# cerbos/cerbos

Measured on NVIDIA H100. Metric: checkresources_decisions_per_sec, higher is better.
Workload: dtype u64

## Files before the change

### cerbos_b200/csrc/cb_core.h

```cpp
#pragma once
#include <stdint.h>
#if !defined(__CUDACC_RTC__)
#include <math.h>
#endif

#include "cerbos_b200_format.h"

#if defined(__CUDACC__)
#define CB_HD __host__ __device__ __forceinline__
#define CB_HD_NOINLINE __host__ __device__ __noinline__
#else
#define CB_HD inline
#define CB_HD_NOINLINE
#endif

namespace cb {

struct alignas(16) U4 { uint32_t x, y, z, w; };

struct TableLayout {
    uint32_t off[32];
    uint32_t nV, nRP, nS, nP, nR, nAP, nT, n_slots, n_rows;
    uint32_t has_role_policies, has_parent_roles, has_principal_policies;
    uint32_t image_bytes;
// ... 39 lines not shown
    CB_HD const U4 *urows() const { return reinterpret_cast<const U4 *>(base + L->uc_rows_off); }
    CB_HD const U4 *uc_chain() const { return reinterpret_cast<const U4 *>(base + L->uc_chain_off); }
};

enum { CB_MAX_GATHER = 8 };
struct BatchView {
    const cb_hdr0 *hdr0;
    const cb_hdr1 *hdr1;
    const uint32_t *roles;
    const uint64_t *slots;
    const uint64_t *heap;
    const uint32_t *bstr_off;
    const uint8_t *bstr_bytes;
    const uint32_t *class_off, *class_pats, *aset_k;
    const uint64_t *aset_spread;
    const uint64_t *row_am;
    uint32_t n_rows;
    uint64_t stride;
    uint64_t first, count;
    uint32_t role_cols, n_asets, kc, n_pass, max_actions, kbytes, flags;
    uint32_t rcp, stride_pattern;
    int64_t now;
    const uint32_t *perm;
    uint32_t prefetch_slots;
    uint32_t *defer_list, *defer_count;
    uint32_t *count_dev;
    uint32_t *tile_counter;
    uint8_t *outs[CB_MAX_GATHER];
    uint32_t n_out;
    uint32_t *sig_flags[CB_MAX_GATHER];
    const uint32_t *wait_flags;
    uint32_t sig_rank, sig_step, wait_step;
    const uint32_t *strpred;
    const U4 *uc_rows_pk;
    uint32_t n_bstr;
    uint64_t heap_words;
};

#ifndef __CUDACC_RTC__
inline void finish_batch_view(BatchView &b) {
    b.perm = nullptr;
    b.prefetch_slots = 0;
    b.defer_list = nullptr; b.defer_count = nullptr; b.count_dev = nullptr; b.tile_counter = nullptr;
    b.n_out = 0;
    for (int i = 0; i < CB_MAX_GATHER; i++) { b.outs[i] = nullptr; b.sig_flags[i] = nullptr; }
    b.wait_flags = nullptr; b.sig_rank = 0; b.sig_step = 0; b.wait_step = 0;
    b.strpred = nullptr;
    b.uc_rows_pk = nullptr;
    b.rcp = 1;
    while (b.rcp < b.role_cols) b.rcp <<= 1;
    b.stride_pattern = 0;
    for (uint32_t j = 0; j * b.role_cols < 32; j++) b.stride_pattern |= 1u << (j * b.role_cols);
}
#endif

template <typename T>
CB_HD T ldg(const T *p) { return *p; }

CB_HD uint64_t ldcol64(const uint64_t *p) {
#if defined(__CUDA_ARCH__)
    uint64_t v;
    asm("ld.global.nc.L1::no_allocate.u64 %0, [%1];" : "=l"(v) : "l"(p));
    return v;
#else
    return *p;
#endif
}
CB_HD uint32_t ldcol32(const uint32_t *p) {
#if defined(__CUDA_ARCH__)
    uint32_t v;
    asm("ld.global.nc.L1::no_allocate.u32 %0, [%1];" : "=r"(v) : "l"(p));
    return v;
#else
    return *p;
#endif
}

CB_HD U4 ld16(const void *p) { return *reinterpret_cast<const U4 *>(p); }
CB_HD U4 ldcol128(const void *p) {
#if defined(__CUDA_ARCH__)
// ... 3478 lines not shown
CB_HD int strpred_tri(const BatchView &b, uint64_t x, uint32_t p) {
#ifdef CB_UC_STUB_STRPRED
    return (int)((x >> p) & 1u);
#endif
    if (v64_bad(x)) return TRI_E;
    if (v64_tag(x) != CB_V64_STRING) return TRI_E;
    return (int)((ldg(b.strpred + (uint32_t)(x & 0xFFFFFFFFu)) >> p) & 1u);
}
CB_HD bool typed_str(uint64_t x) { return (uint32_t)(x >> 32) == (uint32_t)(CB_V64_BOX_BASE | CB_V64_STRING) << 16; }
CB_HD bool typed_num(uint64_t x) { const double d = u2d(x); return v64_tag(x) == 0 && d == d; }
CB_HD bool typed_bool(uint64_t x) { return (x >> 1) == (uint64_t)(CB_V64_BOX_BASE | CB_V64_BOOL) << 47; }
CB_HD bool typed_list(const ListRegs &L, uint32_t need) {
    bool ok = L.st == 0 && L.len >= need;
#ifdef CB_LIST_KEYS64
    for (int j = 0; j < CB_LC; j++) ok &= (uint32_t)j >= L.len || (uint32_t)(L.e[j] >> 48) == (CB_V64_BOX_BASE | CB_V64_STRING);
#endif
    return ok;
}
CB_HD bool uc_typed(bool guard) {
#ifdef CB_UC_STUB_FALLBACK
    return guard || true;
#endif
    return guard;
}
CB_HD uint32_t typed_id(uint64_t key) { return (uint32_t)key; }
CB_HD uint64_t typed_box(uint32_t id) { return ((uint64_t)(CB_V64_BOX_BASE | CB_V64_STRING) << 48) | id; }
CB_HD bool typed_ord(uint32_t ci, double dx, double dy) { return ci == 2 ? dx < dy : ci == 3 ? dx <= dy : ci == 4 ? dx > dy : dx >= dy; }
CB_HD bool typed_strpred(const BatchView &b, uint32_t id, uint32_t p) {
#ifdef CB_UC_STUB_STRPRED
    return ((id >> p) & 1u) != 0;
#endif
    return ((ldg(b.strpred + id) >> p) & 1u) != 0;
}
template <typename Cols>
CB_HD ListKey list_elem_key(const TableView t, const BatchView &b, const Cols &cols, uint32_t v, const ListRegs &L, uint32_t i) {
    if (L.st == 2) return list_probe_key(elem_operand(t, b, cols.slot(v), i));
    return list_probe_key(list_elem(t, b, 0ull, L, i));
}

struct OneCols {
    uint64_t x;
    CB_HD uint64_t slot(uint32_t) const { return x; }
};
CB_HD bool term_lit(int tri, uint32_t flags) { return (flags & CB_TERM_LIT_F) ? tri == TRI_F : tri == TRI_T; }
template <typename Cols>
CB_HD uint32_t flat_dnf_inline(const TableView t, const BatchView &b, const Cols &cols, uint32_t pid, uint32_t flat_off, uint32_t info) {
    const uint32_t nt = info & 0xFFFF;
    const cb_instr *terms = t.code() + flat_off;
    bool any = false, group = true, slow = false;
    for (uint32_t i = 0; i < nt; i++) {
        const U4 w = ld16(terms + 2 * i);
        const uint32_t flags = (w.x >> 8) & 0xFF;
        group &= term_lit(term_tri(t, b, cols, pid, w, slow), flags);
        if (flags & CB_TERM_GROUP_END) { any |= group; group = true; }
    }
    if (slow) return 4u;
    return (uint32_t)(any != (bool)((info >> 24) & 1));
}
template <typename Cols>
CB_HD uint32_t cond_eval(const TableView t, const BatchView &b, const Cols &cols, uint32_t pid, uint32_t gid) {
    U4 cd = ld16(t.conds() + gid);
    if (cd.w) return flat_dnf_inline(t, b, cols, pid, cd.z, cd.w);
    return 4u;
}

CB_HD uint32_t chain_start(const TableView t, uint32_t scope, uint32_t kind_flag, bool lenient) {
// ... 804 lines not shown
```

### cerbos_b200/csrc/cb_specialize.h

```cpp
#pragma once
#include <stdint.h>

#include <cstdio>
#include <cstring>
#include <map>
#include <string>
#include <vector>

#include "cerbos_b200_format.h"

namespace cbspec {

struct Limits {
    uint32_t max_shapes = 8;
    uint32_t max_items = 96;
};

inline std::string hex(uint32_t v) {
    char buf[16];
    snprintf(buf, sizeof buf, "0x%xu", v);
    return buf;
}
inline std::string hex64(uint64_t v) {
    char buf[32];
// ... 582 lines not shown
                break;
            }
            if (op == CB_TERM_STARTS || op == CB_TERM_ENDS || op == CB_TERM_CONTAINS) {
                if (xk == CB_OPK_SLOT) want(w[1], 'S');
                if (yk == CB_OPK_SLOT) want(w[2], 'S');
                break;
            }
            if (xk == CB_OPK_SLOT && yk != CB_OPK_SLOT) want(w[1], tyy);
            if (yk == CB_OPK_SLOT && xk != CB_OPK_SLOT) want(w[2], tx);
            break;
        }
        }
    }
    for (uint32_t v = 0; v < ns && typed; v++) {
        if (slot_list[v]) want(v, 'L');
        if ((slot_used[v] || slot_list[v]) && (!ty[v] || atoms.slot_used[v])) typed = false;
    }
    auto typed_operand = [&](uint32_t kind, uint32_t v, uint32_t aux, char &k) -> std::string {
        const std::string V = std::to_string(v);
        if (kind == CB_OPK_CONST) {
            const uint64_t c = consts[v];
            k = const_type(c);
            if (k == 'S') return hex((uint32_t)c);
            if (k == 'N') return "u2d(" + hex64(c) + ")";
            if (k == 'B') return c & 1u ? "true" : "false";
            return "";
        }
        if (kind == CB_OPK_PID) { k = 'S'; return "pid"; }
        if (kind == CB_OPK_SLOT_SIZE) { k = 'N'; return "(double)cols.l" + V + ".len"; }
        if (kind == CB_OPK_SLOT_ELEM) { k = 'S'; return "typed_id(cols.l" + V + ".e[" + std::to_string(aux) + "])"; }
        k = v < ns && (ty[v] == 'S' || ty[v] == 'N' || ty[v] == 'B') ? ty[v] : 0;
        return k == 'S' ? "typed_id(cols.k" + V + ")" : k == 'N' ? "cols.d" + V : k == 'B' ? "cols.b" + V : "";
    };
    auto typed_term = [&](uint32_t q) -> std::string {
        const uint32_t *w = terms[q].data();
        const uint32_t op = w[0] & 0xFF, flags = (w[0] >> 8) & 0xFF, xk = (w[0] >> 16) & 0xFF, yk = w[0] >> 24, ci = flags & CB_TERM_CI_MASK;
        if (form[q] == 'P') return "typed_strpred(b, typed_id(cols.k" + std::to_string(w[1]) + "), " + std::to_string(pred_of[q]) + "u)";
        if (form[q] == 'L') {
            if (op == CB_TERM_IN_CS || op == CB_TERM_IN_SS || op == CB_TERM_IN) {
                if (probe_of[q] == CB_NONE32) return "";
                if (op == CB_TERM_IN_CS && const_type(consts[w[1]]) == 0) return "";
                if (op == CB_TERM_IN && xk == CB_OPK_CONST && const_type(consts[w[1]]) == 0) return "";
                return "(h" + std::to_string(w[2]) + " & " + hex(1u << probe_of[q]) + ") != 0u";
            }
            const std::string a = std::to_string(mask_of[q].first), bb = std::to_string(mask_of[q].second);
            return op == CB_TERM_SUBSET ? "m" + a + "_" + bb + " == (1u << cols.l" + a + ".len) - 1u" : "m" + a + "_" + bb + " != 0u";
        }
        char kx = 0, ky = 0;
        std::string x, y;
        switch (op) {
        case CB_TERM_EQ_SS: case CB_TERM_ORD_SS:
            x = typed_operand(CB_OPK_SLOT, w[1], 0, kx); y = typed_operand(CB_OPK_SLOT, w[2], 0, ky);
            if (!kx || kx != ky) return "";
            if (op == CB_TERM_EQ_SS) return x + " == " + y;
            return kx == 'N' ? "typed_ord(" + hex(ci) + ", " + x + ", " + y + ")" : "";
        case CB_TERM_EQ_SC: case CB_TERM_ORD_SC:
            x = typed_operand(CB_OPK_SLOT, w[1], 0, kx); y = typed_operand(CB_OPK_CONST, w[2], 0, ky);
            if (!kx || kx != ky) return "";
            if (op == CB_TERM_EQ_SC) return x + " == " + y;
            return kx == 'N' ? "typed_ord(" + hex(ci) + ", " + x + ", " + y + ")" : "";
        case CB_TERM_EQ_SP: return "typed_id(cols.k" + std::to_string(w[1]) + ") == pid";
        case CB_TERM_IN_SC: {
            const uint64_t *p = theap + (consts[w[2]] & 0xFFFFFFFFFFFFull);
            x = typed_operand(CB_OPK_SLOT, w[1], 0, kx);
            if (!kx || kx != in_const_type(q)) return "";
            std::string e;
            for (uint32_t j = 0; j < (uint32_t)p[0]; j++)
                e += std::string(j ? " | " : "") + "(" + x + " == " + (kx == 'S' ? hex((uint32_t)p[1 + j]) : "u2d(" + hex64(p[1 + j]) + ")") + ")";
            return e;
        }
        case CB_TERM_HAS: return "true";
        case CB_TERM_CMP:
            x = typed_operand(xk, w[1], w[3] & 0xFFFFu, kx); y = typed_operand(yk, w[2], w[3] >> 16, ky);
            if (!kx || !ky) return "";
            if (ci == 0) return kx == ky ? x + " == " + y : "false";
            return kx == 'N' && ky == 'N' ? "typed_ord(" + hex(ci) + ", " + x + ", " + y + ")" : "";
        case CB_TERM_STARTS: case CB_TERM_ENDS: case CB_TERM_CONTAINS:
            x = typed_operand(xk, w[1], w[3] & 0xFFFFu, kx); y = typed_operand(yk, w[2], w[3] >> 16, ky);
            if (kx != 'S' || ky != 'S') return "";
            return "str_tri(t, b, " + std::to_string(op) + "u, typed_box(" + x + "), typed_box(" + y + ")) == TRI_T";
        default: return "";
        }
    };
    std::vector<std::string> tterm(terms.size());
    for (uint32_t q = 0; q < terms.size() && typed; q++) {
        tterm[q] = typed_term(q);
        typed = !tterm[q].empty();
    }
    auto probe_key = [&](const Probe &x) -> std::string {
        const std::string V = std::to_string(x.v);
        if (x.kind == CB_OPK_CONST || x.kind == CB_OPK_PID) return "list_probe_key(" + x.value + ")";
        if (x.kind == CB_OPK_SLOT) return x.v < ns && ty[x.v] == 'S' ? "cols.k" + V : "";
        if (x.kind == CB_OPK_SLOT_ELEM) return "list_elem_key(t, b, cols, " + V + "u, cols.l" + V + ", " + std::to_string(x.aux) + "u)";
        return "";
    };
    for (const auto &pl : probes)
        for (const Probe &x : pl.second) typed &= !probe_key(x).empty();
    std::string s;
    s += "// generated by cb_specialize.h (generate_uc) from the loaded table: every distinct condition, straight-line\n";
    s += "namespace cb {\n";
    for (const std::string &a : atoms.src) s += a;
    auto reg = [&](uint32_t v) { return slot_used[v] || slot_list[v]; };
    s += "struct SpecRegs {\n    CachedCols g;\n";
    for (uint32_t v = 0; v < ns; v++)
        if (reg(v)) s += "    uint64_t s" + std::to_string(v) + ";\n";
    if (typed) {
        s += "    bool typed;   // every slot below holds the type its terms compare it as (SpecConds::load)\n";
        for (uint32_t v = 0; v < ns; v++) {
            const std::string V = std::to_string(v);
            if (ty[v] == 'S') s += "    ListKey k" + V + ";   // string: its probe key (the id when typed)\n";
            if (ty[v] == 'N') s += "    double d" + V + ";\n";
            if (ty[v] == 'B') s += "    bool b" + V + ";\n";
        }
    }
    for (uint32_t v = 0; v < ns; v++)
        if (slot_list[v]) s += "    ListRegs l" + std::to_string(v) + ";\n";
    s += "    CB_HD uint64_t slot(uint32_t v) const {\n        switch (v) {\n";
    for (uint32_t v = 0; v < ns && !typed; v++)
        if (reg(v)) s += "        case " + std::to_string(v) + "u: return s" + std::to_string(v) + ";\n";
    s += "        default: return v < " + std::to_string(ns) + "u ? g.slot(v) : (uint64_t)(CB_V64_BOX_BASE | CB_V64_ERROR) << 48;\n        }\n    }\n};\n";
    s += "struct SpecConds {\n    static constexpr uint32_t n_strpred = " + std::to_string(n_pred_bits) + "u;\n";
    s += std::string("    static constexpr int kForm = ") + (n_uconds <= 31 ? "CB_UC_FORM_MASK32" : n_uconds <= 63 ? "CB_UC_FORM_MASK64" : "CB_UC_FORM_INDEX") + ";   // how the rows name their conditions\n";
    s += "    static constexpr uint32_t kScopeRows = " + std::to_string(scope_rows) + "u;   // rows of the longest scope (cb::uc_walk)\n";
    s += std::string("    static constexpr bool kPrograms = ") + (have_atoms ? "true" : "false") + ";   // leaf programs: needs the value helpers of cb_core.h\n";
    s += "    template <typename Cols>\n    CB_HD SpecRegs load(const TableView t, const BatchView &b, const Cols &c) const {\n        SpecRegs r;\n        r.g.b = c.b; r.g.n = c.n;\n";
    for (uint32_t v = 0; v < ns; v++)
        if (reg(v)) s += "        r.s" + std::to_string(v) + " = c.slot(" + std::to_string(v) + "u);\n";
    if (typed) {
        std::string guard;
        for (uint32_t v = 0; v < ns; v++) {
            const std::string V = std::to_string(v);
            if (!reg(v)) continue;
            if (ty[v] == 'L') s += "        r.l" + V + " = list_load(t, b, r.s" + V + ");\n";
            if (ty[v] == 'S') s += "        r.k" + V + " = list_probe_key(r.s" + V + ");\n";
            if (ty[v] == 'N') s += "        r.d" + V + " = u2d(r.s" + V + ");\n";
            if (ty[v] == 'B') s += "        r.b" + V + " = (r.s" + V + " & 1u) != 0;\n";
            guard += std::string(guard.empty() ? "" : " & ") + (ty[v] == 'L' ? "typed_list(r.l" + V + ", " + std::to_string(list_need[v]) + "u)"
                                                                 : std::string(ty[v] == 'S' ? "typed_str" : ty[v] == 'N' ? "typed_num" : "typed_bool") + "(r.s" + V + ")");
        }
        s += "        r.typed = " + guard + ";\n";
    } else {
        for (uint32_t v = 0; v < ns; v++)
            if (slot_list[v]) s += "        r.l" + std::to_string(v) + " = list_load(t, b, r.s" + std::to_string(v) + ");\n";
    }
    s += "        return r;\n    }\n";
    s += "    // the predicate word of one string (pre-pass over the string dictionary; bit p = predicate p holds)\n";
    s += "    CB_HD uint32_t strpred(const TableView t, const BatchView &b, uint32_t id) const {\n";
    s += "        OneCols cols; cols.x = ((uint64_t)(CB_V64_BOX_BASE | CB_V64_STRING) << 48) | id;\n        bool slow = false; uint32_t bits = 0u; const uint32_t pid = 0u;\n";
    for (uint32_t p = 0; p < pred_terms.size(); p++) {
        const uint32_t *w = terms[pred_terms[p]].data();
        s += "        bits |= (uint32_t)(term_tri(t, b, cols, pid, U4{" + hex(w[0]) + ", 0x0u, " + hex(w[2]) + ", " + hex(w[3]) + "}, slow) == TRI_T) << " + std::to_string(p) + ";\n";
    }
    {
        bool any = false;
// ... 61 lines not shown
            continue;
        }
        const uint32_t nt = cd[3] & 0xFFFFu, negate = (cd[3] >> 24) & 1u;
        std::string &c = cond_src[u];
        c += in + "{   // distinct condition " + std::to_string(u) + "\n" + in + "    bool any = false, group = true;\n";
        std::string any, group;
        for (uint32_t i = 0; i < nt; i++) {
            const uint32_t *w = code + 2 * (cd[2] + 2 * i);
            const uint32_t flags = (w[0] >> 8) & 0xFFu;
            const uint32_t q = term_ids[{w[0] & kUseMask, w[1], w[2], w[3]}];
            c += in + "    group &= term_lit(q" + std::to_string(q) + ", " + hex(flags) + ");\n";
            group += std::string(group.empty() ? "" : " & ") + (flags & CB_TERM_LIT_F ? "!t" : "t") + std::to_string(q);
            if (flags & CB_TERM_GROUP_END) {
                c += in + "    any |= group; group = true;\n";
                any += std::string(any.empty() ? "" : " | ") + "(" + group + ")";
                group.clear();
            }
        }
        c += in + "    " + word + std::string(" |= (uint64_t)(any != ") + (negate ? "true" : "false") + ") << " + sh + ";\n" + in + "}\n";
        if (any.empty()) any = "false";
        typed_src += "            " + word + " |= (uint64_t)(" + (negate ? "!(" + any + ")" : any) + ") << " + sh + ";   // condition " + std::to_string(u) + "\n";
    }
    if (typed) {
        s += atom_src + "        CondWord val; val.lo = 1ull; val.hi = 0ull;\n" + typed_src + "        } else {   // the tri-state terms on the slot words, reloaded (cols.slot)\n" + tri;
        for (uint32_t u = 1; u <= n_uconds; u++) if (formula[u].empty()) s += cond_src[u];
        s += "        }\n";
        for (uint32_t u = 1; u <= n_uconds; u++) if (!formula[u].empty()) s += cond_src[u];
    } else {
        s += tri + atom_src + "        CondWord val; val.lo = 1ull; val.hi = 0ull;\n";
        for (uint32_t u = 1; u <= n_uconds; u++) s += cond_src[u];
    }
    s += "        return val;\n    }\n};\n}  // namespace cb\n";
    out.src = s;
    out.n_strpred = n_pred_bits;
    out.n_atoms = (uint32_t)atoms.src.size();
    return out;
}

}
```

### cerbos_b200/csrc/cerbos_b200.cu

```cuda
#include <cuda_runtime.h>
#include <dlfcn.h>
#include <sys/stat.h>
#include <unistd.h>

#include <atomic>
#include <cstdarg>
#include <cstdio>
#include <cstdlib>
#include <cstring>
#include <map>
#include <mutex>
#include <new>
#include <string>
#include <thread>
#include <vector>

#include "cb_core.h"
#include "cb_kernels.h"
#include "cb_specialize.h"
#include "cb_uc.h"
#include "cb_encode.h"
#include "cb_narrow.h"
#include "cb_host.h"
#include "cb_embed.inc"
// ... 317 lines not shown
        while (c < n) c <<= 1;
        T *fresh = nullptr;
        const cudaError_t e = cudaMallocAsync(reinterpret_cast<void **>(&fresh), c * sizeof(T), stream);
        if (e != cudaSuccess) return e;
        T *old = ptr;
        ptr = fresh;
        cap = c;
        return old ? cudaFreeAsync(old, stream) : cudaSuccess;
    }
};

}

struct cgpu_ctx {
    int device = 0;
    int sm_count = 0;
    uint32_t *d_status = nullptr;
    std::atomic<uint64_t> launches{0};
    std::mutex mu;
    std::vector<Slot> slots;
    LaunchPlan last_plan;
    uint32_t last_grid = 0, last_window = 0, last_buckets = 0;
    int force_no_stage = 0;
    int force_general = 0;
    int cluster_mode = -1;
    int force_no_tiles = 0;
    int force_no_jit = 0;
    struct DeferLane {
        uint32_t seq = 0;
        uint32_t *cells = nullptr;
        struct Bufs {
            LaneBuf<uint32_t> list;
            LaneBuf<uint32_t> strpred;
            LaneBuf<cb::U4> pk;
        } q[4];
    };
    std::map<cudaStream_t, DeferLane> defer_lanes;
    std::mutex defer_mu;
    cudaStream_t copy_stream = nullptr;
    cudaEvent_t copy_ev[16] = {};
    uint32_t copy_seq = 0;
    struct SliceUse { const void *ptr; cudaEvent_t done; uint8_t *stage; size_t stage_bytes; };
    std::vector<SliceUse> slice_uses;
    std::mutex copy_mu;
    std::vector<cgpu_ctx *> peers;
    int uc_mode = -1;
    bool profiling = false;
    cudaEvent_t ev0 = nullptr, ev1 = nullptr;
    double prof_ms = 0;
    uint64_t prof_n = 0;
    bool prof_pending = false;
};

struct cgpu_encoder { cbenc::Encoder enc; };
struct cgpu_encoded {
    cbenc::Columns cols;
    void *pinned = nullptr;
    size_t pinned_cap = 0;
    const void *ptrs[CGPU_N_COLUMNS] = {};
    size_t bytes[CGPU_N_COLUMNS] = {};
    uint32_t flags = 0;
    uint32_t n_slots = 0, role_cols = 1;
};
struct cgpu_narrowed {
    cbnarrow::Narrowed nb;
    const cgpu_encoded *enc = nullptr;
// ... 67 lines not shown
}

const char kSpecPrelude[] =
    "#define CB_LEAN_ONLY 1\n"
    "#ifndef CB_SPEC_MIN_BLOCKS\n#define CB_SPEC_MIN_BLOCKS 5\n#endif\n"
    "typedef unsigned char uint8_t; typedef unsigned short uint16_t; typedef unsigned int uint32_t; typedef unsigned long long uint64_t;\n"
    "typedef signed char int8_t; typedef short int16_t; typedef int int32_t; typedef long long int64_t; typedef unsigned long long uintptr_t;\n";
const char kSpecKernels[] =
    "\nextern \"C\" __global__ void __launch_bounds__(256, CB_SPEC_MIN_BLOCKS) cb_spec_tiles(const __grid_constant__ cbk::TableDesc td, const __grid_constant__ cb::BatchView bv,\n"
    "        uint8_t *bitmap, uint8_t *effects, uint32_t *status, const uint32_t n_slots) {\n"
    "    extern __shared__ __align__(128) uint8_t smem_image[];\n"
    "    __shared__ __align__(8) uint64_t mbar_tab, mbar_col[4];\n"
    "    cbk::check_tiles_body<cb::SpecBlocks>(td, bv, bitmap, effects, status, n_slots, smem_image, &mbar_tab, mbar_col);\n"
    "}\n"
    "extern \"C\" __global__ void __launch_bounds__(256, CB_SPEC_MIN_BLOCKS) cb_spec_direct(const __grid_constant__ cbk::TableDesc td, const __grid_constant__ cb::BatchView bv,\n"
    "        uint8_t *bitmap, uint8_t *effects, uint32_t *status, const uint32_t stage_rt) {\n"
    "    extern __shared__ __align__(128) uint8_t smem_image[];\n"
    "    __shared__ __align__(8) uint64_t mbar;\n"
    "    cbk::check_body<true, 1, cb::SpecBlocks>(td, bv, bitmap, effects, status, stage_rt, smem_image, &mbar);\n"
    "}\n";
const char kSpecUcStaged[] =
    "\nextern \"C\" __global__ void __launch_bounds__(256, CB_SPEC_UC_MIN_BLOCKS) cb_spec_uc(const __grid_constant__ cbk::TableDesc td, const __grid_constant__ cb::BatchView bv,\n"
    "        uint8_t *bitmap, uint8_t *effects, uint32_t *status, const uint32_t) {\n"
    "    extern __shared__ __align__(128) uint8_t smem_image[];\n"
    "    __shared__ __align__(8) uint64_t mbar;\n"
    "    cbk::check_uc_body<cb::SpecConds, cb::GlobalCols, true>(td, bv, bitmap, effects, smem_image, &mbar);\n"
    "}\n";
const char kSpecUcGlobal[] =
    "\nextern \"C\" __global__ void __launch_bounds__(256, CB_SPEC_UC_MIN_BLOCKS) cb_spec_uc_global(const __grid_constant__ cbk::TableDesc td, const __grid_constant__ cb::BatchView bv,\n"
    "        uint8_t *bitmap, uint8_t *effects, uint32_t *status, const uint32_t) {\n"
    "    cbk::check_uc_body<cb::SpecConds, cb::GlobalCols, false>(td, bv, bitmap, effects, nullptr, nullptr);\n"
    "}\n";
const char kSpecUcStrpred[] =
    "\nextern \"C\" __global__ void __launch_bounds__(256) cb_spec_strpred(const __grid_constant__ cbk::TableDesc td, const __grid_constant__ cb::BatchView bv, uint32_t *out, const uint32_t n) {\n"
    "    const uint32_t id = blockIdx.x * 256u + threadIdx.x;\n"
    "    cb::TableView tv; tv.base = td.base; tv.L = &td.lay;\n"
    "    if (id < n) out[id] = cb::SpecConds().strpred(tv, bv, id);\n"
    "}\n";

uint64_t fnv1a(const void *p, size_t n, uint64_t h = 1469598103934665603ull) {
    const uint8_t *b = static_cast<const uint8_t *>(p);
    for (size_t i = 0; i < n; i++) { h ^= b[i]; h *= 1099511628211ull; }
    return h;
}
std::string cache_path(uint64_t key) {
    const char *d = getenv("CERBOS_B200_CACHE_DIR");
    std::string dir;
    if (d) { if (!d[0]) return ""; dir = d; }
    else { const char *home = getenv("HOME"); if (!home || !home[0]) return ""; dir = std::string(home) + "/.cache/cerbos_b200"; }
    char name[64];
    snprintf(name, sizeof name, "/spec_%016llx.cubin", (unsigned long long)key);
    return dir + name;
}
bool cache_read(const std::string &path, std::vector<char> *out) {
    if (path.empty()) return false;
    FILE *f = fopen(path.c_str(), "rb");
    if (!f) return false;
    fseek(f, 0, SEEK_END);
    const long n = ftell(f);
    fseek(f, 0, SEEK_SET);
    bool ok = n > 0;
    if (ok) { out->resize((size_t)n); ok = fread(out->data(), 1, (size_t)n, f) == (size_t)n; }
    fclose(f);
    return ok;
}
void cache_write(const std::string &path, const std::vector<char> &data) {
    if (path.empty()) return;
    const std::string dir = path.substr(0, path.rfind('/'));
    for (size_t i = 1; i <= dir.size(); i++)
        if (i == dir.size() || dir[i] == '/') mkdir(dir.substr(0, i).c_str(), 0755);
// ... 132 lines not shown
int launch_cluster(cgpu_ctx *ctx, const cgpu_table *t, const cb::BatchView &bv, uint32_t **perm_out, cudaStream_t stream) {
    const cb::TableLayout &lay = t->desc.lay;
    ClusterParams p{};
    p.hdr0 = bv.hdr0; p.hdr1 = bv.hdr1; p.first = bv.first; p.count = (uint32_t)bv.count;
    p.nV = lay.nV; p.nRP = lay.nRP; p.nS = lay.nS;
    const uint64_t nkeys = (uint64_t)(lay.nV + 1) * (lay.nRP + 1) * (lay.nS + 1);
    p.nb = 32;
    while (p.nb < nkeys && p.nb < kMaxBuckets) p.nb <<= 1;
    const uint64_t per_req = 24 + 4ull * bv.role_cols + 8ull * lay.n_slots + 16;
    uint64_t w = kClusterChunk;
    while (w * 2 * per_req <= kClusterWindowBytes) w <<= 1;
    while (w < 64ull * p.nb && w < (1ull << 22)) w <<= 1;
    p.window = (uint32_t)w;
    const uint32_t n_win = (uint32_t)((bv.count + w - 1) / w);
    const uint32_t n_chunks = (uint32_t)((bv.count + kClusterChunk - 1) / kClusterChunk);
    const size_t perm_bytes = ((size_t)bv.count * 4 + 255) & ~(size_t)255, keys_bytes = ((size_t)bv.count * 2 + 255) & ~(size_t)255;
    const size_t hist_bytes = (size_t)n_win * p.nb * 4;
    uint8_t *scratch = nullptr;
    CUDA_TRY(cudaMallocAsync(reinterpret_cast<void **>(&scratch), perm_bytes + keys_bytes + hist_bytes, stream));
    p.perm = reinterpret_cast<uint32_t *>(scratch);
    p.keys = reinterpret_cast<uint16_t *>(scratch + perm_bytes);
    p.hist = reinterpret_cast<uint32_t *>(scratch + perm_bytes + keys_bytes);
    CUDA_TRY(cudaMemsetAsync(p.hist, 0, hist_bytes, stream));
    cluster_count<<<n_chunks, kThreads, 0, stream>>>(p);
    cluster_scan<<<n_win, kThreads, 0, stream>>>(p);
    cluster_scatter<<<n_chunks, kThreads, 0, stream>>>(p);
    CUDA_TRY(cudaGetLastError());
    ctx->launches.fetch_add(3, std::memory_order_relaxed);
    ctx->last_window = p.window; ctx->last_buckets = p.nb;
    *perm_out = p.perm;
    return CGPU_OK;
}

int acquire_defer(cgpu_ctx *ctx, cudaStream_t stream, uint64_t count, uint32_t **list, uint32_t **cell, size_t n_strpred, uint32_t **strpred,
                  size_t n_pk, cb::U4 **pk) {
    std::lock_guard<std::mutex> g(ctx->defer_mu);
    cgpu_ctx::DeferLane &ln = ctx->defer_lanes[stream];
    if (!ln.cells) {
        CUDA_TRY(cudaMalloc(reinterpret_cast<void **>(&ln.cells), 4 * 16));
        CUDA_TRY(cudaMemset(ln.cells, 0, 4 * 16));
    }
    const uint32_t q = ln.seq++ & 3;
    cgpu_ctx::DeferLane::Bufs &b = ln.q[q];
    CUDA_TRY(b.list.fit(count, 1024, stream));
    if (n_strpred) CUDA_TRY(b.strpred.fit(n_strpred, 4096, stream));
    if (n_pk) CUDA_TRY(b.pk.fit(n_pk, 4096, stream));
    *list = b.list.ptr;
    *cell = ln.cells + 4 * q;
    *strpred = n_strpred ? b.strpred.ptr : nullptr;
    *pk = n_pk ? b.pk.ptr : nullptr;
    return CGPU_OK;
}

LaunchPlan plan_launch(const cgpu_ctx &ctx, const cgpu_table &t, const cb::BatchView &bv) {
    const cb::TableLayout &lay = t.desc.lay;
    LaunchPlan p;
    p.stage = !ctx.force_no_stage && lay.image_bytes <= kMaxStageBytes;
    const bool spec_ready = t.spec_state.load(std::memory_order_acquire) == 1;
    const bool uc_spec_ready = spec_ready && t.spec_uc_global != nullptr;
    const bool mostly_programs = t.uc.ok && !uc_spec_ready && 2 * (uint64_t)t.uc.n_gids_flat < t.uc.n_gids;
    p.lean = !ctx.force_general && !mostly_programs && cbhost::lean_eligible(lay, t.meta, bv);
    const uint64_t n_pk = (uint64_t)bv.n_asets * lay.n_rows;
    p.uc = p.lean && cbhost::uc_eligible(lay, t.uc, bv) && (uc_spec_ready || !t.uc.needs_spec()) && t.d_uc_image &&
           (ctx.uc_mode == 1 || (ctx.uc_mode != 0 && ctx.cluster_mode != 1 && t.meta[CB_META_BLOCK_SHAPES] > 1));
    p.cluster = !p.uc && bv.count < (1ull << 32) &&
                (ctx.cluster_mode == 1 || (ctx.cluster_mode != 0 && bv.count >= kClusterMinRequests && t.meta[CB_META_BLOCK_SHAPES] > 1));
    const uint32_t tile_bytes = cb::tile_cols_bytes(bv.role_cols, lay.n_slots);
    const uint64_t small_tabs = n_pk * 8 + (((uint64_t)bv.n_asets + 1) & ~1ull) * 4 + 16 + 2 * kThreads;
    const uint32_t tiles_smem = ((lay.image_bytes + 127u) & ~127u) + 2 * tile_bytes + (uint32_t)(small_tabs < 65536 ? small_tabs : 65536);
    auto al16 = [](const void *ptr) { return (reinterpret_cast<uintptr_t>(ptr) & 15) == 0; };
    p.col_tiles = !p.uc && p.lean && p.stage && !p.cluster && !ctx.force_no_tiles && tiles_smem <= kMaxTilesSmem && bv.stride % 4 == 0 &&
                  bv.first % 4 == 0 && al16(bv.hdr0) && al16(bv.hdr1) && al16(bv.roles) && al16(bv.slots);
    p.uc_staged = p.uc && !ctx.force_no_stage && uc_stageable(t.uc, n_pk) && (!uc_spec_ready || t.spec_uc != nullptr);
    p.spec = p.uc ? uc_spec_ready : p.lean && p.stage && bv.count < (1ull << 32) && spec_ready && t.spec_tiles != nullptr;
    p.kernel = p.uc        ? (p.spec ? (p.uc_staged ? Kernel::SpecUc : Kernel::SpecUcGlobal) : p.uc_staged ? Kernel::Uc : Kernel::UcGlobal)
             : p.spec      ? (p.col_tiles ? Kernel::SpecTiles : Kernel::SpecDirect)
             : p.col_tiles ? Kernel::LeanTiles
             : p.lean      ? (p.stage ? Kernel::Lean : Kernel::LeanGlobal)
                           : (p.stage ? Kernel::General : Kernel::GeneralGlobal);
    p.smem = p.uc ? (p.uc_staged ? (uint32_t)uc_smem_bytes(t.uc, n_pk) : 0) : p.col_tiles ? tiles_smem : p.stage ? lay.image_bytes : 0;
    p.last_arg = p.col_tiles ? lay.n_slots : p.stage ? 1u : 0u;
    p.serialise = p.spec && !p.uc && !ctx.profiling;
// ... 39 lines not shown
cudaError_t launch_serialised(const void *fn, uint32_t grid, uint32_t block, uint32_t smem, cudaStream_t stream, void **args) {
    cudaLaunchConfig_t cfg = {};
    cfg.gridDim = dim3(grid); cfg.blockDim = dim3(block); cfg.dynamicSmemBytes = smem; cfg.stream = stream;
    cudaLaunchAttribute pdl[1];
    pdl[0].id = cudaLaunchAttributeProgrammaticStreamSerialization;
    pdl[0].val.programmaticStreamSerializationAllowed = 1;
    cfg.attrs = pdl; cfg.numAttrs = 1;
    return cudaLaunchKernelExC(&cfg, fn, args);
}

int launch_check(cgpu_ctx *ctx, const cgpu_table *t, const LaunchPlan &plan, const cb::BatchView &bv, uint8_t *d_bitmap, uint8_t *d_effects,
                 uint32_t *d_status, cudaStream_t stream) {
    const cb::TableLayout &lay = t->desc.lay;
    const uint64_t tiles = (bv.count + kThreads - 1) / kThreads;
    const int occ = resident_ctas(*t, plan.kernel, plan.smem);
    if (occ < 0) return occ;
    const uint64_t max_ctas = (uint64_t)ctx->sm_count * (uint64_t)occ;
    uint32_t grid = (uint32_t)(tiles < max_ctas ? tiles : max_ctas);
    if (grid == 0) grid = 1;
    TableDesc td = plan.uc ? t->uc_desc : t->desc;
    cb::BatchView bvv = bv;
    bvv.perm = nullptr;
    bvv.prefetch_slots = lay.n_slots <= 8 ? lay.n_slots : 0;
    uint32_t *perm = nullptr;
    if (plan.cluster) {
        int rc = launch_cluster(ctx, t, bv, &perm, stream);
        if (rc != CGPU_OK) return rc;
        bvv.perm = perm;
    }
    uint32_t last_arg = plan.last_arg;
    uint32_t *defer = nullptr;
    if (plan.lean) {
        uint32_t *cell = nullptr, *strpred = nullptr;
        cb::U4 *pk = nullptr;
        const uint32_t n_str = lay.nT + bv.n_bstr;
        const uint64_t n_pk = (uint64_t)bv.n_asets * lay.n_rows;
        int rc = acquire_defer(ctx, stream, bv.count, &defer, &cell, plan.strpred ? (size_t)n_str + 1 : 0, &strpred, plan.merge_rows ? (size_t)n_pk : 0, &pk);
        if (rc != CGPU_OK) return rc;
        if (plan.merge_rows) {
            uc_merge_rows<<<(unsigned)((n_pk + kThreads - 1) / kThreads), kThreads, 0, stream>>>(t->uc_desc, bvv, pk, (uint32_t)n_pk);
            CUDA_TRY(cudaGetLastError());
            ctx->launches.fetch_add(1, std::memory_order_relaxed);
            bvv.uc_rows_pk = pk;
        }
        bvv.defer_count = cell;
        bvv.tile_counter = plan.col_tiles ? cell + 2 : nullptr;
        bvv.defer_list = defer;
        if (plan.strpred && n_str) {
            TableDesc ptd = t->uc_desc;
            uint32_t n_arg = n_str;
            void *pargs[] = {&ptd, &bvv, &strpred, &n_arg};
            CUDA_TRY(cudaLaunchKernel((const void *)t->spec_strpred, dim3((n_str + 255) / 256), dim3(256), pargs, 0, stream));
            ctx->launches.fetch_add(1, std::memory_order_relaxed);
        }
        bvv.strpred = strpred;
    }
    const void *fn = kernel_fn(*t, plan.kernel);
    void *args[] = {&td, &bvv, &d_bitmap, &d_effects, &d_status, &last_arg};
    if (ctx->profiling) {
        if (ctx->prof_pending && cudaEventSynchronize(ctx->ev1) == cudaSuccess) {
            float ms = 0;
            if (cudaEventElapsedTime(&ms, ctx->ev0, ctx->ev1) == cudaSuccess) { ctx->prof_ms += ms; ctx->prof_n++; }
            ctx->prof_pending = false;
        }
        CUDA_TRY(cudaEventRecord(ctx->ev0, stream));
    }
    if (plan.serialise) {
        CUDA_TRY(launch_serialised(fn, grid, kThreads, plan.smem, stream, args));
    } else {
        CUDA_TRY(cudaLaunchKernel(fn, dim3(grid), dim3(kThreads), args, plan.smem, stream));
    }
    CUDA_TRY(cudaGetLastError());
    if (ctx->profiling) { CUDA_TRY(cudaEventRecord(ctx->ev1, stream)); ctx->prof_pending = true; }
    if (plan.lean) {
        cb::BatchView dv = bv;
        dv.perm = defer;
        dv.count_dev = bvv.defer_count;
        dv.prefetch_slots = 0;
        const Kernel gk = plan.stage ? Kernel::General : Kernel::GeneralGlobal;
        const uint32_t gsmem = plan.stage ? lay.image_bytes : 0;
        const int gocc = resident_ctas(*t, gk, gsmem);
        if (gocc < 0) return gocc;
        const uint64_t gmax = (uint64_t)ctx->sm_count;
        const uint32_t ggrid = (uint32_t)(tiles < gmax ? tiles : gmax);
        uint32_t stage_arg = plan.stage ? 1u : 0u;
        TableDesc gtd = t->desc;
        void *gargs[] = {&gtd, &dv, &d_bitmap, &d_effects, &d_status, &stage_arg};
        CUDA_TRY(launch_serialised(kernel_fn(*t, gk), ggrid ? ggrid : 1, kThreads, gsmem, stream, gargs));
// ... 61 lines not shown
    const char *nt = getenv("CERBOS_B200_NO_TILES");
    ctx->force_no_tiles = nt && nt[0] == '1';
    const char *um = getenv("CERBOS_B200_UC");
    ctx->uc_mode = um && (um[0] == '0' || um[0] == '1') ? um[0] - '0' : -1;
    const char *cm = getenv("CERBOS_B200_CLUSTER");
    ctx->cluster_mode = cm && (cm[0] == '0' || cm[0] == '1') ? cm[0] - '0' : -1;
    cudaMemPool_t pool;
    if (cudaDeviceGetDefaultMemPool(&pool, ctx->device) == cudaSuccess) {
        uint64_t keep = ~0ull;
        cudaMemPoolSetAttribute(pool, cudaMemPoolAttrReleaseThreshold, &keep);
    }
    ctx->slots.resize(4);
    *out = ctx;
    return CGPU_OK;
}

void cgpu_shutdown(cgpu_ctx *ctx) {
    if (!ctx) return;
    for (cgpu_ctx *p : ctx->peers) cgpu_shutdown(p);
    ctx->peers.clear();
    cudaSetDevice(ctx->device);
    cudaDeviceSynchronize();
    for (auto &s : ctx->slots) {
        if (s.stream) cudaStreamDestroy(s.stream);
        if (s.h2d) cudaStreamDestroy(s.h2d);
        if (s.d2h) cudaStreamDestroy(s.d2h);
        for (auto e : s.ev) cudaEventDestroy(e);
        if (s.dev) cudaFree(s.dev);
        if (s.h_status) cudaFreeHost(s.h_status);
        if (s.d_status) cudaFree(s.d_status);
    }
    if (ctx->d_status) cudaFree(ctx->d_status);
    for (auto &kv : ctx->defer_lanes) {
        for (auto &b : kv.second.q) { cudaFree(b.list.ptr); cudaFree(b.strpred.ptr); cudaFree(b.pk.ptr); }
        if (kv.second.cells) cudaFree(kv.second.cells);
    }
    if (ctx->copy_stream) cudaStreamDestroy(ctx->copy_stream);
    for (auto e : ctx->copy_ev) if (e) cudaEventDestroy(e);
    for (auto &u : ctx->slice_uses) { if (u.done) cudaEventDestroy(u.done); if (u.stage) cudaFree(u.stage); }
    if (ctx->ev0) cudaEventDestroy(ctx->ev0);
    if (ctx->ev1) cudaEventDestroy(ctx->ev1);
    delete ctx;
}

int cgpu_table_load(cgpu_ctx *ctx, const void *blob, size_t len, cgpu_table **out) {
    if (!ctx || !out) return fail(CGPU_ERR_INVALID, "cgpu_table_load: null argument");
    *out = nullptr;
    cgpu_table *t = new (std::nothrow) cgpu_table();
    if (!t) return fail(CGPU_ERR_INVALID, "out of memory");
    t->ctx = ctx;
    int rc = invalid(cbhost::parse_blob(blob, len, &t->desc.lay, t->meta, t->sec_len));
    if (rc != CGPU_OK) { delete t; return rc; }
    t->uc = cbuc::build(static_cast<const uint8_t *>(blob), t->desc.lay.off, t->sec_len, t->meta, t->desc.lay);
    cudaError_t e = cudaSetDevice(ctx->device);
    if (e == cudaSuccess) e = cudaMalloc(reinterpret_cast<void **>(&t->d_image), t->desc.lay.image_bytes);
    if (e == cudaSuccess) e = cudaMemcpy(t->d_image, blob, t->desc.lay.image_bytes, cudaMemcpyHostToDevice);
    if (e == cudaSuccess && t->uc.ok) {
        e = cudaMalloc(reinterpret_cast<void **>(&t->d_uc_image), t->uc.bytes.size());
        if (e == cudaSuccess) e = cudaMemcpy(t->d_uc_image, t->uc.bytes.data(), t->uc.bytes.size(), cudaMemcpyHostToDevice);
    }
    if (e != cudaSuccess) {
        if (t->d_image) cudaFree(t->d_image);
        if (t->d_uc_image) cudaFree(t->d_uc_image);
        delete t;
        return fail(CGPU_ERR_CUDA, "table upload failed: %s", cudaGetErrorString(e));
    }
    t->desc.base = t->d_image;
// ... 748 lines not shown
```

Measured before the change: 87.33 billion.

## Precompute per-string affix records for slot-vs-slot startsWith/endsWith terms

Adds a per-string 16-byte record (length plus first and last four bytes), built by the strpred prepass kernel and stored in a new lane buffer. The specialized typed path for startsWith/endsWith between two slot strings now checks short needles with a couple of masked compares on these records instead of calling str_tri. Needles longer than four bytes still fall back to the full comparison. The cost is an extra buffer and extra work in the prepass, and the strpred prepass is now forced on whenever records are needed.

```diff
diff --git a/cerbos_b200/csrc/cb_core.h b/cerbos_b200/csrc/cb_core.h
--- a/cerbos_b200/csrc/cb_core.h
+++ b/cerbos_b200/csrc/cb_core.h
@@ -95,6 +95,7 @@
     const uint32_t *wait_flags;
     uint32_t sig_rank, sig_step, wait_step;
     const uint32_t *strpred;
+    const U4 *strrec;
     const U4 *uc_rows_pk;
     uint32_t n_bstr;
     uint64_t heap_words;
@@ -109,6 +110,7 @@
     for (int i = 0; i < CB_MAX_GATHER; i++) { b.outs[i] = nullptr; b.sig_flags[i] = nullptr; }
     b.wait_flags = nullptr; b.sig_rank = 0; b.sig_step = 0; b.wait_step = 0;
     b.strpred = nullptr;
+    b.strrec = nullptr;
     b.uc_rows_pk = nullptr;
     b.rcp = 1;
     while (b.rcp < b.role_cols) b.rcp <<= 1;
@@ -3653,6 +3655,31 @@
 #endif
     return ((ldg(b.strpred + id) >> p) & 1u) != 0;
 }
+CB_HD U4 str_record(const TableView t, const BatchView &b, uint32_t id) {
+    const StrRef s = str_ref(t, b, typed_box(id));
+    U4 r;
+    r.x = s.len; r.y = 0u; r.z = 0u; r.w = 0u;
+    for (uint32_t j = 0; j < 4u && j < s.len; j++) {
+        r.y |= (uint32_t)ldg(s.p + j) << (8u * j);
+        r.z |= (uint32_t)ldg(s.p + s.len - 1u - j) << (8u * (3u - j));
+    }
+    return r;
+}
+CB_HD U4 str_rec(const TableView t, const BatchView &b, uint32_t id) {
+#if defined(__CUDA_ARCH__)
+    (void)t;
+    return ld16(b.strrec + id);
+#else
+    return b.strrec ? ld16(b.strrec + id) : str_record(t, b, id);
+#endif
+}
+CB_HD bool typed_affix(const TableView t, const BatchView &b, uint32_t op, uint32_t x, uint32_t y) {
+    const U4 a = str_rec(t, b, x), c = str_rec(t, b, y);
+    if (c.x > a.x) return false;
+    if (c.x > 4u) return str_tri(t, b, op, typed_box(x), typed_box(y)) == TRI_T;
+    if (op == CB_TERM_STARTS) return ((a.y ^ c.y) & (c.x == 4u ? ~0u : (1u << (8u * c.x)) - 1u)) == 0u;
+    return ((a.z ^ c.z) & (c.x == 0u ? 0u : ~0u << (8u * (4u - c.x)))) == 0u;
+}
 template <typename Cols>
 CB_HD ListKey list_elem_key(const TableView t, const BatchView &b, const Cols &cols, uint32_t v, const ListRegs &L, uint32_t i) {
     if (L.st == 2) return list_probe_key(elem_operand(t, b, cols.slot(v), i));
diff --git a/cerbos_b200/csrc/cb_specialize.h b/cerbos_b200/csrc/cb_specialize.h
--- a/cerbos_b200/csrc/cb_specialize.h
+++ b/cerbos_b200/csrc/cb_specialize.h
@@ -638,6 +638,7 @@
         k = v < ns && (ty[v] == 'S' || ty[v] == 'N' || ty[v] == 'B') ? ty[v] : 0;
         return k == 'S' ? "typed_id(cols.k" + V + ")" : k == 'N' ? "cols.d" + V : k == 'B' ? "cols.b" + V : "";
     };
+    bool str_recs = false;
     auto typed_term = [&](uint32_t q) -> std::string {
         const uint32_t *w = terms[q].data();
         const uint32_t op = w[0] & 0xFF, flags = (w[0] >> 8) & 0xFF, xk = (w[0] >> 16) & 0xFF, yk = w[0] >> 24, ci = flags & CB_TERM_CI_MASK;
@@ -684,6 +685,10 @@
         case CB_TERM_STARTS: case CB_TERM_ENDS: case CB_TERM_CONTAINS:
             x = typed_operand(xk, w[1], w[3] & 0xFFFFu, kx); y = typed_operand(yk, w[2], w[3] >> 16, ky);
             if (kx != 'S' || ky != 'S') return "";
+            if (op != CB_TERM_CONTAINS && xk == CB_OPK_SLOT && yk == CB_OPK_SLOT) {
+                str_recs = true;
+                return "typed_affix(t, b, " + std::to_string(op) + "u, " + x + ", " + y + ")";
+            }
             return "str_tri(t, b, " + std::to_string(op) + "u, typed_box(" + x + "), typed_box(" + y + ")) == TRI_T";
         default: return "";
         }
@@ -725,7 +730,10 @@
     for (uint32_t v = 0; v < ns && !typed; v++)
         if (reg(v)) s += "        case " + std::to_string(v) + "u: return s" + std::to_string(v) + ";\n";
     s += "        default: return v < " + std::to_string(ns) + "u ? g.slot(v) : (uint64_t)(CB_V64_BOX_BASE | CB_V64_ERROR) << 48;\n        }\n    }\n};\n";
-    s += "struct SpecConds {\n    static constexpr uint32_t n_strpred = " + std::to_string(n_pred_bits) + "u;\n";
+    const bool recs = typed && str_recs;
+    const uint32_t n_strpred = recs && n_pred_bits == 0 ? 1u : n_pred_bits;
+    s += "struct SpecConds {\n    static constexpr uint32_t n_strpred = " + std::to_string(n_strpred) + "u;\n";
+    s += std::string("    static constexpr bool kStrRecs = ") + (recs ? "true" : "false") + ";   // typed_affix reads BatchView::strrec\n";
     s += std::string("    static constexpr int kForm = ") + (n_uconds <= 31 ? "CB_UC_FORM_MASK32" : n_uconds <= 63 ? "CB_UC_FORM_MASK64" : "CB_UC_FORM_INDEX") + ";   // how the rows name their conditions\n";
     s += "    static constexpr uint32_t kScopeRows = " + std::to_string(scope_rows) + "u;   // rows of the longest scope (cb::uc_walk)\n";
     s += std::string("    static constexpr bool kPrograms = ") + (have_atoms ? "true" : "false") + ";   // leaf programs: needs the value helpers of cb_core.h\n";
@@ -853,7 +861,7 @@
     }
     s += "        return val;\n    }\n};\n}  // namespace cb\n";
     out.src = s;
-    out.n_strpred = n_pred_bits;
+    out.n_strpred = n_strpred;
     out.n_atoms = (uint32_t)atoms.src.size();
     return out;
 }
diff --git a/cerbos_b200/csrc/cerbos_b200.cu b/cerbos_b200/csrc/cerbos_b200.cu
--- a/cerbos_b200/csrc/cerbos_b200.cu
+++ b/cerbos_b200/csrc/cerbos_b200.cu
@@ -373,6 +373,7 @@
         struct Bufs {
             LaneBuf<uint32_t> list;
             LaneBuf<uint32_t> strpred;
+            LaneBuf<cb::U4> strrec;
             LaneBuf<cb::U4> pk;
         } q[4];
     };
@@ -506,10 +507,12 @@
     "    cbk::check_uc_body<cb::SpecConds, cb::GlobalCols, false>(td, bv, bitmap, effects, nullptr, nullptr);\n"
     "}\n";
 const char kSpecUcStrpred[] =
-    "\nextern \"C\" __global__ void __launch_bounds__(256) cb_spec_strpred(const __grid_constant__ cbk::TableDesc td, const __grid_constant__ cb::BatchView bv, uint32_t *out, const uint32_t n) {\n"
+    "\nextern \"C\" __global__ void __launch_bounds__(256) cb_spec_strpred(const __grid_constant__ cbk::TableDesc td, const __grid_constant__ cb::BatchView bv, uint32_t *out,\n"
+    "        cb::U4 *rec, const uint32_t n) {\n"
     "    const uint32_t id = blockIdx.x * 256u + threadIdx.x;\n"
     "    cb::TableView tv; tv.base = td.base; tv.L = &td.lay;\n"
     "    if (id < n) out[id] = cb::SpecConds().strpred(tv, bv, id);\n"
+    "    if (cb::SpecConds::kStrRecs && id < n) rec[id] = cb::str_record(tv, bv, id);\n"
     "}\n";
 
 uint64_t fnv1a(const void *p, size_t n, uint64_t h = 1469598103934665603ull) {
@@ -708,7 +711,7 @@
     return CGPU_OK;
 }
 
-int acquire_defer(cgpu_ctx *ctx, cudaStream_t stream, uint64_t count, uint32_t **list, uint32_t **cell, size_t n_strpred, uint32_t **strpred,
+int acquire_defer(cgpu_ctx *ctx, cudaStream_t stream, uint64_t count, uint32_t **list, uint32_t **cell, size_t n_strpred, uint32_t **strpred, cb::U4 **strrec,
                   size_t n_pk, cb::U4 **pk) {
     std::lock_guard<std::mutex> g(ctx->defer_mu);
     cgpu_ctx::DeferLane &ln = ctx->defer_lanes[stream];
@@ -720,10 +723,12 @@
     cgpu_ctx::DeferLane::Bufs &b = ln.q[q];
     CUDA_TRY(b.list.fit(count, 1024, stream));
     if (n_strpred) CUDA_TRY(b.strpred.fit(n_strpred, 4096, stream));
+    if (n_strpred) CUDA_TRY(b.strrec.fit(n_strpred, 1024, stream));
     if (n_pk) CUDA_TRY(b.pk.fit(n_pk, 4096, stream));
     *list = b.list.ptr;
     *cell = ln.cells + 4 * q;
     *strpred = n_strpred ? b.strpred.ptr : nullptr;
+    *strrec = n_strpred ? b.strrec.ptr : nullptr;
     *pk = n_pk ? b.pk.ptr : nullptr;
     return CGPU_OK;
 }
@@ -829,10 +834,10 @@
     uint32_t *defer = nullptr;
     if (plan.lean) {
         uint32_t *cell = nullptr, *strpred = nullptr;
-        cb::U4 *pk = nullptr;
+        cb::U4 *pk = nullptr, *strrec = nullptr;
         const uint32_t n_str = lay.nT + bv.n_bstr;
         const uint64_t n_pk = (uint64_t)bv.n_asets * lay.n_rows;
-        int rc = acquire_defer(ctx, stream, bv.count, &defer, &cell, plan.strpred ? (size_t)n_str + 1 : 0, &strpred, plan.merge_rows ? (size_t)n_pk : 0, &pk);
+        int rc = acquire_defer(ctx, stream, bv.count, &defer, &cell, plan.strpred ? (size_t)n_str + 1 : 0, &strpred, &strrec, plan.merge_rows ? (size_t)n_pk : 0, &pk);
         if (rc != CGPU_OK) return rc;
         if (plan.merge_rows) {
             uc_merge_rows<<<(unsigned)((n_pk + kThreads - 1) / kThreads), kThreads, 0, stream>>>(t->uc_desc, bvv, pk, (uint32_t)n_pk);
@@ -846,11 +851,12 @@
         if (plan.strpred && n_str) {
             TableDesc ptd = t->uc_desc;
             uint32_t n_arg = n_str;
-            void *pargs[] = {&ptd, &bvv, &strpred, &n_arg};
+            void *pargs[] = {&ptd, &bvv, &strpred, &strrec, &n_arg};
             CUDA_TRY(cudaLaunchKernel((const void *)t->spec_strpred, dim3((n_str + 255) / 256), dim3(256), pargs, 0, stream));
             ctx->launches.fetch_add(1, std::memory_order_relaxed);
         }
         bvv.strpred = strpred;
+        bvv.strrec = strrec;
     }
     const void *fn = kernel_fn(*t, plan.kernel);
     void *args[] = {&td, &bvv, &d_bitmap, &d_effects, &d_status, &last_arg};
@@ -978,7 +984,7 @@
     }
     if (ctx->d_status) cudaFree(ctx->d_status);
     for (auto &kv : ctx->defer_lanes) {
-        for (auto &b : kv.second.q) { cudaFree(b.list.ptr); cudaFree(b.strpred.ptr); cudaFree(b.pk.ptr); }
+        for (auto &b : kv.second.q) { cudaFree(b.list.ptr); cudaFree(b.strpred.ptr); cudaFree(b.strrec.ptr); cudaFree(b.pk.ptr); }
         if (kv.second.cells) cudaFree(kv.second.cells);
     }
     if (ctx->copy_stream) cudaStreamDestroy(ctx->copy_stream);
```

After: 88.82 billion, median of 6. +1.7%, better.
